# benihime91/pytorch_retinanet

Measured on AMD Instinct MI355X. Metric: images/sec RetinaNet-R50-FPN train step @800x1333, higher is better.
Workload: dtype bf16; 1 GPU; RetinaNet-R50-FPN bf16 train step, per-GPU batch 8 x 3x800x1333 (padded 800x1344), A=201600 anchors, K=90, T=8 GT/img, SGD(momentum, fp32 masters + bf16 conv weights); random-init weights; global_batch=8, parallelism=dp1

## Files before the change

### pytorch_retinanet_amd/csrc/conv.hip

```cpp
#include "rn_common.hpp"
#include <type_traits>
#include <cstdlib>

#ifndef BAND_NARROW_FWD
#define BAND_NARROW_FWD 1
#endif

namespace {

using rn::f32x16;
typedef __attribute__((address_space(3))) void *lds_void_ptr;

constexpr int CONV_BM = 256, CONV_BN = 256, CONV_BK = 64, CONV_THREADS = 512;
constexpr int CONV_LDS_BYTES = 5 * CONV_BM * CONV_BK * 2;
#define SWZ(row) (((row) >> 1) & 7)

constexpr int CONV_MAX_PROBLEMS = 4;

constexpr int CONV_LEVELS = 6;
struct LevelSet {
    const int32_t *map;
    int32_t row_elems, slots, n_images, T;
    int32_t hw[CONV_LEVELS];
    uint16_t *ptr[CONV_LEVELS];
};

__device__ __forceinline__ void sheet_coords(const int m, const int HWp, int &n, int &pos)
{
    n = (int)(((float)m + 0.5f) * (1.0f / (float)HWp));
    pos = m - n * HWp;
}

struct LevelRegs { uint32_t lo[CONV_LEVELS], hi[CONV_LEVELS]; int32_t hw[CONV_LEVELS]; };
__device__ __forceinline__ LevelRegs level_regs(const LevelSet &ls)
{
    LevelRegs r;
#pragma unroll
    for (int l = 0; l < CONV_LEVELS; ++l) {
        const unsigned long long u = (unsigned long long)(uintptr_t)ls.ptr[l];
        r.lo[l] = __builtin_amdgcn_readfirstlane((uint32_t)u);
        r.hi[l] = __builtin_amdgcn_readfirstlane((uint32_t)(u >> 32));
        r.hw[l] = __builtin_amdgcn_readfirstlane(ls.hw[l]);
    }
    return r;
}

__device__ __forceinline__ uint16_t *level_row(const LevelSet &ls, const LevelRegs &lr, const int n, const int32_t e)
{
    if (e < 0) return nullptr;
    const int t = (e >> 24) & 15, img = n * ls.slots + ((e >> 28) & 7), local = e & 0xffffff;
    uint32_t lo = lr.lo[0], hi = lr.hi[0];
    int hw = lr.hw[0];
#pragma unroll
    for (int l = 1; l < CONV_LEVELS; ++l) {
        lo = t == l ? lr.lo[l] : lo;
        hi = t == l ? lr.hi[l] : hi;
        hw = t == l ? lr.hw[l] : hw;
    }
    if (t >= ls.T || img >= ls.n_images || local >= hw) return nullptr;
    uint16_t *base = (uint16_t *)(uintptr_t)(((unsigned long long)hi << 32) | lo);
    return base + ((int64_t)img * hw + local) * ls.row_elems;
}

__device__ __forceinline__ void map_fetch(int32_t &dst, const int32_t *p) { asm volatile("global_load_dword %0, %1, off" : "=v"(dst) : "v"(p) : "memory"); }
__device__ __forceinline__ void map_landed(int32_t &dst) { asm volatile("" : "+v"(dst) :: "memory"); }

__device__ __forceinline__ const uint16_t *bperm_ptr(const uint16_t *p, const int src_lane)
{
    const unsigned long long u = (unsigned long long)(uintptr_t)p;
    unsigned lo, hi;
    const unsigned sel = (unsigned)src_lane << 2;
    asm volatile("ds_bpermute_b32 %0, %2, %3\n\tds_bpermute_b32 %1, %2, %4\n\ts_waitcnt lgkmcnt(0)"
                 : "=&v"(lo), "=&v"(hi) : "v"(sel), "v"((unsigned)u), "v"((unsigned)(u >> 32)) : "memory");
    return (const uint16_t *)(uintptr_t)(((unsigned long long)hi << 32) | lo);
}
template <int LANE_A, int LANE_B>
__device__ __forceinline__ const uint16_t *pair_ptr(const uint16_t *p, const bool second)
{
    const unsigned long long u = (unsigned long long)(uintptr_t)p;
    const unsigned lo_a = __builtin_amdgcn_readlane((unsigned)u, LANE_A), hi_a = __builtin_amdgcn_readlane((unsigned)(u >> 32), LANE_A);
    const unsigned lo_b = __builtin_amdgcn_readlane((unsigned)u, LANE_B), hi_b = __builtin_amdgcn_readlane((unsigned)(u >> 32), LANE_B);
    const unsigned long long a = ((unsigned long long)hi_a << 32) | lo_a, b = ((unsigned long long)hi_b << 32) | lo_b;
    return (const uint16_t *)(uintptr_t)(second ? b : a);
}

enum { MODE_CANVAS = 0, MODE_TO_LEVELS = 1, MODE_FROM_LEVELS = 2, MODE_DENSE = 3 };
struct DenseGeom {
    int64_t M[CONV_MAX_PROBLEMS];
    int32_t h[CONV_MAX_PROBLEMS], w[CONV_MAX_PROBLEMS];
    int32_t tile_beg[CONV_MAX_PROBLEMS + 1];
};

struct ConvArgs {
    const uint16_t *Xs[CONV_MAX_PROBLEMS];
    const uint16_t *Ws[CONV_MAX_PROBLEMS];
    const float *biases[CONV_MAX_PROBLEMS];
    uint16_t *Ys[CONV_MAX_PROBLEMS];
    const uint8_t *mask;
    const uint16_t *zeros;
    const uint8_t *relu_masks[CONV_MAX_PROBLEMS];
    float *colsums[CONV_MAX_PROBLEMS];
    uint8_t *relu_mask_outs[CONV_MAX_PROBLEMS];
    int64_t M, HWp;
    int Cin, Cout, Wp, relu;
    int n_base;
    int f16;
    LevelSet lv;
    DenseGeom dn;
    int ksplit;
    float *kpartial;
    int xcd_ny, xcd_q, xcd_r;
    const uint16_t *X2s[CONV_MAX_PROBLEMS];
    int x_split, x_ld;
};
struct ConvProblem { const uint16_t *X, *W; const float *bias; uint16_t *Y; };

struct Walk { int tap, chunk; };

template <int DT, int MODE, bool NARROW = false>
__global__ __launch_bounds__(CONV_THREADS) void conv3x3_canvas_kernel(const ConvArgs args)
{
    constexpr int MI = NARROW ? 1 : 4;
    int prob = blockIdx.z, bx = blockIdx.x, by = blockIdx.y;
    if (args.xcd_ny > 0) {
        const int xcd = bx & 7, w = bx >> 3, mt = w / args.xcd_ny;
        by = w - mt * args.xcd_ny;
        if (mt >= args.xcd_q + (xcd < args.xcd_r)) return;
        bx = xcd * args.xcd_q + (xcd < args.xcd_r ? xcd : args.xcd_r) + mt;
    }
    int64_t m0 = (int64_t)bx * CONV_BM, M = args.M, HWp = args.HWp;
    int Wp = args.Wp, dense_h = 0;
    if (MODE == MODE_DENSE) {
        prob = 0;
#pragma unroll
        for (int p = 1; p < CONV_MAX_PROBLEMS; ++p) prob = bx >= args.dn.tile_beg[p] ? p : prob;
        m0 = (int64_t)(bx - args.dn.tile_beg[prob]) * CONV_BM;
        M = args.dn.M[prob]; Wp = args.dn.w[prob]; dense_h = args.dn.h[prob]; HWp = (int64_t)Wp * dense_h;
    }
    ConvProblem a;
    a.X = args.Xs[prob]; a.W = args.Ws[prob]; a.bias = args.biases[prob]; a.Y = args.Ys[prob];
    extern __shared__ __attribute__((aligned(16))) unsigned char lds[];
    const int tid = threadIdx.x, lane = tid & 63;
    const int wave = __builtin_amdgcn_readfirstlane(tid >> 6);
    const int wm = NARROW ? wave : wave >> 2, wn = NARROW ? 0 : wave & 3;
    const int grp = wave >> 2;
    const int n0 = by * CONV_BN + args.n_base;
    const int cpt = args.Cin / CONV_BK, KT_ALL = 9 * cpt;
    int kt0 = 0, KT = KT_ALL;
    if (MODE == MODE_DENSE && args.ksplit > 1) {
        const int z = blockIdx.z;
        kt0 = z * KT_ALL / args.ksplit;
        KT = (z + 1) * KT_ALL / args.ksplit - kt0;
    }
    constexpr int TILE = CONV_BM * CONV_BK * 2;
    unsigned char *const Abase = lds, *const Bbase = lds + 3 * TILE;
    auto advance = [&](Walk &w) {
        if (MODE == MODE_FROM_LEVELS) { if (++w.chunk == cpt) { w.chunk = 0; ++w.tap; } }
        else { if (++w.tap == 9) { w.tap = 0; ++w.chunk; } }
    };

    constexpr int MT = 2 * MI, NT = 4;
    rn::f32x4 acc[MT][NT];
#pragma unroll
    for (int i = 0; i < MT; ++i)
#pragma unroll
        for (int j = 0; j < NT; ++j)
#pragma unroll
            for (int r = 0; r < 4; ++r) acc[i][j][r] = 0.0f;

    uint32_t a_off[2], b_off[2];
#pragma unroll
    for (int ks = 0; ks < 2; ++ks) {
        const int chunk = ks * 4 + (lane >> 4);
        { const int row = wm * (32 * MI) + (lane & 15); a_off[ks] = row * 128 + ((chunk ^ SWZ(row)) << 4); }
        { const int row = wn * 64 + (lane & 15); b_off[ks] = row * 128 + ((chunk ^ SWZ(row)) << 4); }
    }
    const uint32_t lds_base = (uint32_t)(uintptr_t)lds;

    const uint16_t *grow[4] = {nullptr, nullptr, nullptr, nullptr};
    LevelRegs lregs = {};
    if (MODE == MODE_TO_LEVELS || MODE == MODE_FROM_LEVELS) lregs = level_regs(args.lv);
    int g_n = 0, g_pos = 0;
    int32_t g_entry = -1;
    bool g_valid = false;
    auto tap_pos = [&](const int t) { return g_pos + (t / 3 - 1) * Wp + (t % 3 - 1); };
    if (MODE == MODE_FROM_LEVELS) {
        const int j = lane & 31;
        int64_t m = m0 + (j >> 3) * 64 + wave * 8 + (j & 7);
        m = m < M ? m : M - 1;
        sheet_coords((int)m, (int)HWp, g_n, g_pos);
        const int p0 = tap_pos(0);
        g_valid = p0 >= 0 && p0 < (int)HWp;
        g_entry = args.lv.map[g_valid ? p0 : 0];
    }
    auto gather_tap = [&](const int t) {
        const uint16_t *mine = level_row(args.lv, lregs, g_n, g_valid ? g_entry : -1);
        const int pn = tap_pos(t + 1 < 9 ? t + 1 : t);
        g_valid = pn >= 0 && pn < (int)HWp;
        map_fetch(g_entry, args.lv.map + (g_valid ? pn : 0));
#pragma unroll
        for (int i = 0; i < 4; ++i) grow[i] = bperm_ptr(mine, i * 8 + (lane >> 3));
    };
    uint32_t voff_a[4], voff_b[4];
#pragma unroll
    for (int i = 0; i < 4; ++i) {
        const int q = i * CONV_THREADS + tid, row = q >> 3, cp = q & 7;
        voff_a[i] = (uint32_t)(row * (MODE == MODE_CANVAS && args.x_split > 0 ? args.x_ld : args.Cin) + ((cp ^ SWZ(row)) << 3)) * 2u;
        voff_b[i] = (uint32_t)(row * 9 * args.Cin + ((cp ^ SWZ(row)) << 3)) * 2u;
    }
    const bool a_edge = m0 - (Wp + 1) < 0 || m0 + CONV_BM + Wp + 1 > M;
    uint32_t tap_ok[4] = {0u, 0u, 0u, 0u};
    if (MODE == MODE_DENSE) {
#pragma unroll
        for (int i = 0; i < 4; ++i) {
            const int64_t m = m0 + ((i * CONV_THREADS + tid) >> 3);
            if (m < M) {
                const int yl = (int)m / Wp, x = (int)m - yl * Wp, y = yl % dense_h;
#pragma unroll
                for (int t = 0; t < 9; ++t)
                    tap_ok[i] |= ((unsigned)(y + t / 3 - 1) < (unsigned)dense_h && (unsigned)(x + t % 3 - 1) < (unsigned)Wp) ? 1u << t : 0u;
            }
        }
    }
    const bool b_ragged = MODE == MODE_TO_LEVELS && n0 + CONV_BN > args.Cout;
    auto lds_piece = [&](unsigned char *stage_base, const int i) {
        return stage_base + i * (CONV_THREADS * 16) + wave * (RN_WAVE * 16);
    };
    auto piece_a = [&](const Walk w, const int stage, const int i) {
        const int c0 = w.chunk * CONV_BK, t = w.tap;
        const int q = i * CONV_THREADS + tid, row = q >> 3, cp = q & 7;
        unsigned char *const sb = Abase + stage * TILE;
        if (MODE == MODE_FROM_LEVELS) {
            const int e = c0 + ((cp ^ SWZ(row)) << 3);
            const int es = e + 8 > args.lv.row_elems ? args.lv.row_elems - 8 : e;
            const uint16_t *g = (grow[i] && e < args.lv.row_elems) ? grow[i] + es : args.zeros + ((cp ^ SWZ(row)) << 3);
            __builtin_amdgcn_global_load_lds((const void *)g, (lds_void_ptr)lds_piece(sb, i), 16, 0, 0);
        } else {
            const int off = (t / 3 - 1) * Wp + (t % 3 - 1);
            if (MODE == MODE_DENSE) {
                const unsigned char *base = (const unsigned char *)a.X + ((m0 + off) * args.Cin + c0) * 2;
                const void *src = (tap_ok[i] >> t) & 1u ? (const void *)(base + voff_a[i]) : (const void *)args.zeros;
                __builtin_amdgcn_global_load_lds(src, (lds_void_ptr)lds_piece(sb, i), 16, 0, 0);
            } else {
                const uint16_t *X = a.X;
                int ld = args.Cin, cs = c0;
                if (MODE == MODE_CANVAS && args.x_split > 0) {
                    ld = args.x_ld;
                    if (w.chunk >= args.x_split) { X = args.X2s[prob]; cs = c0 - args.x_split * CONV_BK; }
                }
                if (!a_edge) {
                    const unsigned char *base = (const unsigned char *)X + ((m0 + off) * ld + cs) * 2;
                    __builtin_amdgcn_global_load_lds((const void *)(base + voff_a[i]), (lds_void_ptr)lds_piece(sb, i), 16, 0, 0);
                } else {
                    int64_t m = m0 + row + off;
                    m = m < 0 ? 0 : (m >= M ? M - 1 : m);
                    const uint16_t *g = X + m * ld + cs + ((cp ^ SWZ(row)) << 3);
                    __builtin_amdgcn_global_load_lds((const void *)g, (lds_void_ptr)lds_piece(sb, i), 16, 0, 0);
                }
            }
        }
    };
    auto piece_b = [&](const Walk w, const int stage, const int i) {
        if (NARROW && i > 0) return;
        const int c0 = w.chunk * CONV_BK, t = w.tap;
        unsigned char *const sb = Bbase + stage * TILE;
        if (!b_ragged) {
            const unsigned char *base = (const unsigned char *)a.W + (((int64_t)n0 * 9 + t) * args.Cin + c0) * 2;
            __builtin_amdgcn_global_load_lds((const void *)(base + voff_b[i]), (lds_void_ptr)lds_piece(sb, i), 16, 0, 0);
        } else {
            const int q = i * CONV_THREADS + tid, row = q >> 3, cp = q & 7;
            const uint16_t *g = a.W + ((int64_t)(n0 + row) * 9 + t) * args.Cin + c0 + ((cp ^ SWZ(row)) << 3);
            if (n0 + row >= args.Cout) g = args.zeros + ((cp ^ SWZ(row)) << 3);
            __builtin_amdgcn_global_load_lds((const void *)g, (lds_void_ptr)lds_piece(sb, i), 16, 0, 0);
        }
    };
    typename rn::mma<DT>::frag fa[MT], fb[NT];
#define RN_DS_READ(dst, addr, OFF) asm volatile("ds_read_b128 %0, %1 offset:" #OFF : "=v"(dst) : "v"(addr))
#define RN_LOAD_FRAGS_AT(AA, KS)                                                   \
    { const uint32_t ba = bbase + b_off[KS], aa = (AA);                            \
      RN_DS_READ(fb[0], ba, 0); RN_DS_READ(fb[1], ba, 2048); RN_DS_READ(fb[2], ba, 4096); RN_DS_READ(fb[3], ba, 6144); \
      RN_DS_READ(fa[0], aa, 0); RN_DS_READ(fa[1], aa, 2048);                        \
      if (MT == 8) { RN_DS_READ(fa[MT - 6], aa, 4096); RN_DS_READ(fa[MT - 5], aa, 6144); RN_DS_READ(fa[MT - 4], aa, 8192);   \
                     RN_DS_READ(fa[MT - 3], aa, 10240); RN_DS_READ(fa[MT - 2], aa, 12288); RN_DS_READ(fa[MT - 1], aa, 14336); } }
#define RN_LOAD_FRAGS(KS) RN_LOAD_FRAGS_AT(abase + a_off[KS], KS)
#define RN_MFMA_ALL()                                                              \
    _Pragma("unroll") for (int mi = 0; mi < MT; ++mi)                              \
        _Pragma("unroll") for (int ni = 0; ni < NT; ++ni)                          \
            acc[mi][ni] = rn::mma<DT>::m16(fa[mi], fb[ni], acc[mi][ni]);
#define RN_MFMA_PHASE()                                                            \
    asm volatile("s_waitcnt lgkmcnt(0)" ::: "memory"); __builtin_amdgcn_sched_barrier(0);          \
    __builtin_amdgcn_s_setprio(1);                                                 \
    RN_MFMA_ALL()                                                                  \
    __builtin_amdgcn_s_setprio(0);                                                 \
    __builtin_amdgcn_sched_barrier(0);                                             \
    __builtin_amdgcn_s_barrier();

    Walk wa = {0, 0}, wb = {0, 0};
    if (MODE == MODE_DENSE) { wa.tap = wb.tap = kt0 % 9; wa.chunk = wb.chunk = kt0 / 9; }
    int sa = 0;
    if (MODE == MODE_FROM_LEVELS) gather_tap(0);
#pragma unroll
    for (int i = 0; i < 4; ++i) piece_a(wa, 0, i);
#pragma unroll
    for (int i = 0; i < 4; ++i) piece_b(wb, 0, i);
    advance(wa); advance(wb);
    if (MODE == MODE_FROM_LEVELS && cpt == 1) {
        asm volatile("s_waitcnt vmcnt(8)" ::: "memory");
        map_landed(g_entry);
        gather_tap(1);
    }
#pragma unroll
    for (int i = 0; i < 4; ++i) piece_a(wa, 1, i);
    advance(wa);
    sa = 2;
    asm volatile("s_waitcnt vmcnt(4)" ::: "memory");
    if (MODE == MODE_FROM_LEVELS) map_landed(g_entry);
    __builtin_amdgcn_s_barrier();
    if (grp == 1) __builtin_amdgcn_s_barrier();


    float bias_pre[4] = {0.0f, 0.0f, 0.0f, 0.0f};
    uint32_t keep[16];
#pragma unroll
    for (int i = 0; i < 16; ++i) keep[i] = 1;
    auto epilogue_prefetch = [&]() {
#pragma unroll
        for (int ni = 0; ni < 4; ++ni) {
            const int col = wn * 64 + ni * 16 + (lane & 15);
            bias_pre[ni] = (a.bias && (MODE != MODE_TO_LEVELS || n0 + col < args.Cout)) ? a.bias[n0 + col] : 0.0f;
        }
        if (MODE != MODE_TO_LEVELS && args.mask) {
            const int64_t pos0 = (int64_t)((uint32_t)m0 % (uint32_t)HWp);
            const bool one_wrap = HWp >= CONV_BM;
#pragma unroll
            for (int i = 0; i < 16; ++i) {
                const int row = i * 16 + (tid >> 5);
                int64_t pos = pos0 + row;
                if (one_wrap) pos = pos >= HWp ? pos - HWp : pos; else pos = (int64_t)((uint32_t)pos % (uint32_t)HWp);
                keep[i] = args.mask[pos];
            }
        }
    };
    int scur = 0;
    for (int kt = 0; kt < KT; ++kt) {
        const uint32_t abase = lds_base + (uint32_t)(scur * TILE), bbase = lds_base + (uint32_t)(3 * TILE + (kt & 1) * TILE);
        scur = scur == 2 ? 0 : scur + 1;
        RN_LOAD_FRAGS(0)
        __builtin_amdgcn_sched_barrier(0);
        if (kt + 1 < KT) {
#pragma unroll
            for (int i = 0; i < 4; ++i) piece_b(wb, (kt + 1) & 1, i);
            advance(wb);
        }
        if (kt == 0) epilogue_prefetch();
        __builtin_amdgcn_sched_barrier(0);
        __builtin_amdgcn_s_barrier();
        RN_MFMA_PHASE()
        RN_LOAD_FRAGS(1)
        __builtin_amdgcn_sched_barrier(0);
        if (kt + 2 < KT) {
            if (MODE == MODE_FROM_LEVELS && wa.chunk == 0) gather_tap(wa.tap);
#pragma unroll
            for (int i = 0; i < 4; ++i) piece_a(wa, sa, i);
            advance(wa);
            sa = sa == 2 ? 0 : sa + 1;
            asm volatile("s_waitcnt vmcnt(4)" ::: "memory");
            if (MODE == MODE_FROM_LEVELS) map_landed(g_entry);
        } else {
            asm volatile("s_waitcnt vmcnt(0)" ::: "memory");
        }
        __builtin_amdgcn_sched_barrier(0);
        __builtin_amdgcn_s_barrier();
        RN_MFMA_PHASE()
    }

#undef RN_DS_READ
#undef RN_LOAD_FRAGS
#undef RN_LOAD_FRAGS_AT
#undef RN_MFMA_ALL
#undef RN_MFMA_PHASE
    if (grp == 0) __builtin_amdgcn_s_barrier();

    if (MODE == MODE_DENSE && args.ksplit > 1) {
        float *__restrict__ out = args.kpartial + ((int64_t)blockIdx.z * M + m0) * args.Cout + n0;
#pragma unroll
        for (int mi = 0; mi < MT; ++mi)
#pragma unroll
            for (int ni = 0; ni < NT; ++ni) {
                const int col = wn * 64 + ni * 16 + (lane & 15);
#pragma unroll
                for (int r = 0; r < 4; ++r) {
                    const int row = wm * (32 * MI) + mi * 16 + 4 * (lane >> 4) + r;
                    if (m0 + row < M) out[(int64_t)row * args.Cout + col] = acc[mi][ni][r];
                }
            }
        return;
    }
    __syncthreads();
    uint16_t *Ys = (uint16_t *)lds;
    uint16_t **Yrow = (uint16_t **)(lds + CONV_BM * CONV_BN * 2);
    float *s_cs = (float *)(lds + CONV_BM * CONV_BN * 2 + 2048);
    uint8_t *s_rmask = lds + CONV_BM * CONV_BN * 2 + 2048 + 16384;
    uint4 *s_lut = (uint4 *)(lds + CONV_BM * CONV_BN * 2 + 2048 + 16384 + 8192);
    static_assert(CONV_BM * CONV_BN * 2 + 2048 + 16384 + 8192 + 4096 <= CONV_LDS_BYTES, "epilogue LDS");
    const uint8_t *relu_mask = MODE == MODE_TO_LEVELS ? nullptr : args.relu_masks[prob];
    uint4 rm_pre = make_uint4(0, 0, 0, 0);
    if (relu_mask) {
        const int row = tid >> 1, half = tid & 1;
        if (m0 + row < M) rm_pre = *(const uint4 *)(relu_mask + (m0 + row) * (args.Cout >> 3) + (n0 >> 3) + half * 16);
    }
    typedef short s16x2 __attribute__((ext_vector_type(2)));
    uint32_t relu_floor = (args.relu & 1) ? 0u : 0x80008000u;
    asm volatile("" : "+v"(relu_floor));
#pragma unroll
    for (int mi = 0; mi < MT; ++mi)
#pragma unroll
        for (int ni = 0; ni < NT; ++ni) {
            const int col = wn * 64 + ni * 16 + (lane & 15);
            const float b = bias_pre[ni];
#pragma unroll
            for (int r = 0; r < 4; r += 2) {
                const int row = wm * (32 * MI) + mi * 16 + 4 * (lane >> 4) + r;
                const float x0 = acc[mi][ni][r] + b, x1 = acc[mi][ni][r + 1] + b;
                uint32_t raw;
                if (DT == RN_BF16) asm("v_cvt_pk_bf16_f32 %0, %1, %2" : "=v"(raw) : "v"(x0), "v"(x1));
                else raw = rn::dt<DT>::pk(x0, x1);
                const uint32_t pk = __builtin_bit_cast(uint32_t, __builtin_elementwise_max(__builtin_bit_cast(s16x2, raw), __builtin_bit_cast(s16x2, relu_floor)));
                Ys[row * CONV_BN + col] = (uint16_t)pk;
                Ys[(row + 1) * CONV_BN + col] = (uint16_t)(pk >> 16);
            }
        }
    if (MODE == MODE_TO_LEVELS && tid < CONV_BM) {
        const int64_t m = m0 + tid;
        uint16_t *dst = nullptr;
        if (m < M) {
            int n, pos;
            sheet_coords((int)m, (int)HWp, n, pos);
            dst = level_row(args.lv, lregs, n, args.lv.map[pos]);
        }
        Yrow[tid] = dst;
    }
    if (relu_mask) {
        *(uint4 *)(s_rmask + tid * 16) = rm_pre;
        if (tid < 256) {
            uint32_t w[4];
#pragma unroll
            for (int j = 0; j < 4; ++j) w[j] = ((tid >> (2 * j)) & 1 ? 0x0000ffffu : 0u) | ((tid >> (2 * j + 1)) & 1 ? 0xffff0000u : 0u);
            s_lut[tid] = make_uint4(w[0], w[1], w[2], w[3]);
        }
    }
    __syncthreads();
    if (MODE == MODE_TO_LEVELS) {
        const int ncols = min(CONV_BN, args.Cout - n0);
#pragma unroll
        for (int i = 0; i < (NARROW ? 4 : 16); ++i) {
            const int q = i * CONV_THREADS + tid, row = NARROW ? q >> 3 : q >> 5, piece = NARROW ? q & 7 : q & 31;
            uint16_t *dst = Yrow[row];
            if (dst && piece * 8 < ncols) {
                const uint16_t *src = Ys + row * CONV_BN + piece * 8;
                dst += n0 + piece * 8;
                if (piece * 8 + 8 <= ncols) {
                    const rn::u32x4 v = *(const rn::u32x4 *)src;
                    asm volatile("global_store_dwordx4 %0, %1, off" :: "v"(dst), "v"(v) : "memory");
                } else {
                    for (int e = 0; e < ncols - piece * 8; e += 2) *(uint32_t *)(dst + e) = *(const uint32_t *)(src + e);
                }
            }
        }
    } else {
        uint8_t *rmask_out = MODE == MODE_TO_LEVELS ? nullptr : args.relu_mask_outs[prob];
        float cs[8] = {0.0f, 0.0f, 0.0f, 0.0f, 0.0f, 0.0f, 0.0f, 0.0f};
#pragma unroll
        for (int i = 0; i < 16; ++i) {
            const int q = i * CONV_THREADS + tid, row = q >> 5, piece = q & 31;
            const int64_t m = m0 + row;
            if (m < M) {
                uint4 v = *(const uint4 *)(Ys + row * CONV_BN + piece * 8);
                if (!keep[i]) v = make_uint4(0, 0, 0, 0);
                if (relu_mask) {
                    const uint4 mk = s_lut[s_rmask[row * 32 + piece]];
                    uint32_t vw[4] = {v.x & mk.x, v.y & mk.y, v.z & mk.z, v.w & mk.w};
#pragma unroll
                    for (int j = 0; j < 4; ++j) {
                        cs[2 * j] += rn::mma<DT>::lo(vw[j]);
                        cs[2 * j + 1] += rn::mma<DT>::hi(vw[j]);
                    }
                    v = make_uint4(vw[0], vw[1], vw[2], vw[3]);
                }
                if (rmask_out) {
                    typedef unsigned short us2 __attribute__((ext_vector_type(2)));
                    const uint32_t vw[4] = {v.x, v.y, v.z, v.w};
                    uint32_t bits = 0;
#pragma unroll
                    for (int j = 0; j < 4; ++j) {
                        const uint32_t nz = __builtin_bit_cast(uint32_t, __builtin_elementwise_min(__builtin_bit_cast(us2, vw[j]), us2{1, 1}));
                        bits |= ((nz | (nz >> 15)) & 3u) << (2 * j);
                    }
                    rmask_out[m * (args.Cout >> 3) + (n0 >> 3) + piece] = (uint8_t)bits;
                }
                *(uint4 *)(a.Y + m * args.Cout + n0 + piece * 8) = v;
            }
        }
        if (relu_mask) {
#pragma unroll
            for (int j = 0; j < 8; ++j) s_cs[(tid >> 5) * CONV_BN + (tid & 31) * 8 + j] = cs[j];
            __syncthreads();
            if (tid < CONV_BN) {
                float t = 0.0f;
#pragma unroll
                for (int r = 0; r < 16; ++r) t += s_cs[r * CONV_BN + tid];
                args.colsums[prob][(int64_t)bx * args.Cout + n0 + tid] = t;
            }
        }
    }
}


constexpr int BAND_BYTES = (CONV_BM + 8) * 128;
constexpr int BANDW_BYTES = 3 * 64 * 128;
constexpr int BAND_LDS = 2 * BAND_BYTES + 2 * BANDW_BYTES;

template <int DT>
__global__ __launch_bounds__(CONV_THREADS) void conv3x3_band_narrow_kernel(const ConvArgs args)
{
    extern __shared__ __attribute__((aligned(16))) unsigned char lds[];
    const int tid = threadIdx.x, lane = tid & 63;
    const int wave = __builtin_amdgcn_readfirstlane(tid >> 6);
    const int64_t m0 = (int64_t)blockIdx.x * CONV_BM, M = args.M;
    const int Wp = args.Wp, cpt = args.Cin / CONV_BK, NB = 3 * cpt;
    const int n0 = args.n_base;
    const uint16_t *__restrict__ X = args.Xs[0], *__restrict__ Wt = args.Ws[0];
    const LevelRegs lregs = level_regs(args.lv);
    const uint32_t lds_base = (uint32_t)(uintptr_t)lds;

    rn::f32x4 acc[2][4];
#pragma unroll
    for (int i = 0; i < 2; ++i)
#pragma unroll
        for (int j = 0; j < 4; ++j)
#pragma unroll
            for (int r = 0; r < 4; ++r) acc[i][j][r] = 0.0f;

    uint32_t a_off[3][2][2], b_off[2];
#pragma unroll
    for (int ks = 0; ks < 2; ++ks) {
        const int chunk = ks * 4 + (lane >> 4);
#pragma unroll
        for (int sft = 0; sft < 3; ++sft)
#pragma unroll
            for (int mi = 0; mi < 2; ++mi) {
                const int row = wave * 32 + mi * 16 + (lane & 15) + sft;
                a_off[sft][mi][ks] = row * 128 + ((chunk ^ SWZ(row)) << 4);
            }
        { const int row = lane & 15; b_off[ks] = row * 128 + ((chunk ^ SWZ(row)) << 4); }
    }

    auto stage = [&](const int b) {
        const int c0 = (b / 3) * CONV_BK, r = b % 3;
        const int64_t p0 = m0 + (int64_t)(r - 1) * Wp - 1;
        unsigned char *const ab = lds + (b & 1) * BAND_BYTES, *const wb = lds + 2 * BAND_BYTES + (b & 1) * BANDW_BYTES;
#pragma unroll
        for (int i = 0; i < 4; ++i) {
            const int q = i * CONV_THREADS + tid, j = q >> 3, cp = q & 7;
            int64_t p = p0 + j;
            p = p < 0 ? 0 : (p >= M ? M - 1 : p);
            const uint16_t *g = X + p * args.Cin + c0 + ((cp ^ SWZ(j)) << 3);
            __builtin_amdgcn_global_load_lds((const void *)g, (lds_void_ptr)(ab + i * (CONV_THREADS * 16) + wave * (RN_WAVE * 16)), 16, 0, 0);
        }
        if (wave == 0) {
            const int j = 256 + (lane >> 3), cp = lane & 7;
            int64_t p = p0 + j;
// ... 878 lines not shown
            rn::dt<DT>::unpack(xv[sr * a.V + j], f0);
#pragma unroll
            for (int e = 0; e < 8; ++e) acc[e] += f0[e];
        }
#pragma unroll
        for (int e = 0; e < 8; ++e) s_acc[(g * a.V + j) * 8 + e] = acc[e];
    }
    __syncthreads();
    const int E = a.V * 8;
    for (int c = t; c < a.C; c += blockDim.x) {
        float tot = 0.0f;
        for (int gg = 0; gg < a.G; ++gg)
            for (int r = 0; r < a.S; ++r) tot += s_acc[gg * E + r * a.C + c];
        if (blockIdx.x == 0)
            for (int64_t row = srows * a.S; row < a.rows[l]; ++row) tot += rn::dt<DT>::ld(x, row * a.C + c);
        a.partial[((int64_t)l * gridDim.x + blockIdx.x) * a.C + c] = tot;
    }
}

__global__ __launch_bounds__(256) void colsum_reduce_kernel(const float *__restrict__ partial, const int tiles, const int C, float *out0,
                                                            float *out1, float *out2, float *out3)
{
    __shared__ double sh[32][8];
    const int p = blockIdx.y, ch = threadIdx.x & 7, ln = threadIdx.x >> 3;
    const int c = blockIdx.x * 8 + ch;
    const float *src = partial + (int64_t)p * tiles * C;
    double s = 0.0;
    if (c < C) {
        int b = ln;
        for (; b + 96 < tiles; b += 128) {
            float v[4];
#pragma unroll
            for (int u = 0; u < 4; ++u) v[u] = src[(int64_t)(b + 32 * u) * C + c];
#pragma unroll
            for (int u = 0; u < 4; ++u) s += (double)v[u];
        }
        for (; b < tiles; b += 32) s += (double)src[(int64_t)b * C + c];
    }
    sh[ln][ch] = s;
    __syncthreads();
    if (ln == 0 && c < C) {
        double t = 0.0;
        for (int l = 0; l < 32; ++l) t += sh[l][ch];
        float *out = p == 0 ? out0 : (p == 1 ? out1 : (p == 2 ? out2 : out3));
        out[c] = (float)t;
    }
}

}

#ifndef CONV_XCD_MAP
#define CONV_XCD_MAP 1
#endif
template <int DT, int MODE, bool NARROW>
static int conv_launch_dt(const ConvArgs &a, const dim3 grid, hipStream_t st)
{
    if (MODE != MODE_DENSE && (a.M >= ((int64_t)1 << 31) || a.HWp >= ((int64_t)1 << 31))) return RN_EUNSUPPORTED;
    static rn::DynLdsOptIn opt_in = {};
    { const int rc = opt_in.ensure((const void *)conv3x3_canvas_kernel<DT, MODE, NARROW>, CONV_LDS_BYTES); if (rc != RN_OK) return rc; }
    if (CONV_XCD_MAP && grid.x >= 16) {
        ConvArgs b = a;
        b.xcd_ny = (int)grid.y; b.xcd_q = (int)(grid.x / 8); b.xcd_r = (int)(grid.x % 8);
        hipLaunchKernelGGL((conv3x3_canvas_kernel<DT, MODE, NARROW>), dim3(8u * (unsigned)(b.xcd_q + (b.xcd_r > 0)) * grid.y, 1, grid.z), dim3(CONV_THREADS),
                           CONV_LDS_BYTES, st, b);
    } else
    hipLaunchKernelGGL((conv3x3_canvas_kernel<DT, MODE, NARROW>), grid, dim3(CONV_THREADS), CONV_LDS_BYTES, st, a);
    RN_LAUNCH_CHECK();
    return RN_OK;
}
template <int MODE, bool NARROW = false>
static int conv_launch_mode(const ConvArgs &a, const dim3 grid, hipStream_t st)
{
    return a.f16 ? conv_launch_dt<RN_F16, MODE, NARROW>(a, grid, st) : conv_launch_dt<RN_BF16, MODE, NARROW>(a, grid, st);
}
static inline bool conv_dtype_ok(const int dtype) { return dtype == RN_BF16 || dtype == RN_F16; }

static int fill_levels(LevelSet &ls, const rn_canvas_layout *lay, int row_elems, void *const *ptrs, int N, int Hp, int Wp)
{
    if (!lay || !lay->map || !ptrs || row_elems <= 0 || (row_elems & 1)) return RN_EINVAL;
    if (lay->T <= 0 || lay->slots <= 0 || lay->n_images <= 0 || (int64_t)N * lay->slots < lay->n_images) return RN_EINVAL;
    if (lay->T > CONV_LEVELS || lay->slots > 8) return RN_EUNSUPPORTED;
    ls.map = lay->map; ls.row_elems = row_elems; ls.slots = lay->slots; ls.n_images = lay->n_images; ls.T = lay->T;
    for (int l = 0; l < CONV_LEVELS; ++l) {
        const int q = l < lay->T ? l : 0;
        if (!ptrs[q] || lay->hw[q] <= 0 || lay->hw[q] >= (1 << 24) || lay->hw[q] > Hp * Wp) return RN_EINVAL;
        if (!rn::aligned(ptrs[q], 16)) return RN_EALIGN;
        if ((int64_t)lay->n_images * lay->hw[q] >= (1ll << 31)) return RN_EUNSUPPORTED;
        ls.hw[l] = lay->hw[q];
        ls.ptr[l] = (uint16_t *)ptrs[q];
    }
    return RN_OK;
}

RN_API int rn_conv3x3_canvas_batched_ex(const void *const *xs, const void *const *ws, const float *const *biases,
                                        const uint8_t *mask, void *const *ys, uint8_t *const *relu_mask_outs, int P, int dtype, int64_t M,
                                        int64_t HWp, int Wp, int Cin, int Cout, int relu, void *stream);

RN_API int rn_conv3x3_canvas_batched(const void *const *xs, const void *const *ws, const float *const *biases,
                                     const uint8_t *mask, void *const *ys, int P, int dtype, int64_t M, int64_t HWp, int Wp,
                                     int Cin, int Cout, int relu, void *stream)
{
    return rn_conv3x3_canvas_batched_ex(xs, ws, biases, mask, ys, nullptr, P, dtype, M, HWp, Wp, Cin, Cout, relu, stream);
}

RN_API int rn_conv3x3_canvas_batched_ex(const void *const *xs, const void *const *ws, const float *const *biases,
                                        const uint8_t *mask, void *const *ys, uint8_t *const *relu_mask_outs, int P, int dtype, int64_t M,
                                        int64_t HWp, int Wp, int Cin, int Cout, int relu, void *stream)
{
    if (relu_mask_outs && !relu) return RN_EINVAL;
    if (!xs || !ws || !ys || P <= 0 || P > CONV_MAX_PROBLEMS || M <= 0 || HWp <= 0 || Wp <= 0 || Cin <= 0 || Cout <= 0) return RN_EINVAL;
    if (!conv_dtype_ok(dtype) || Cin % CONV_BK || Cout % CONV_BN) return RN_EUNSUPPORTED;
    ConvArgs a = {};
    a.f16 = dtype == RN_F16;
    for (int p = 0; p < CONV_MAX_PROBLEMS; ++p) {
        const int q = p < P ? p : 0;
        if (!xs[q] || !ws[q] || !ys[q]) return RN_EINVAL;
        if (!rn::aligned(xs[q], 16) || !rn::aligned(ws[q], 16) || !rn::aligned(ys[q], 16)) return RN_EALIGN;
        a.Xs[p] = (const uint16_t *)xs[q]; a.Ws[p] = (const uint16_t *)ws[q]; a.Ys[p] = (uint16_t *)ys[q];
        a.biases[p] = biases ? biases[q] : nullptr;
        a.relu_mask_outs[p] = relu_mask_outs ? relu_mask_outs[q] : nullptr;
        if (relu_mask_outs && (!relu_mask_outs[q] || !rn::aligned(relu_mask_outs[q], 16))) return relu_mask_outs[q] ? RN_EALIGN : RN_EINVAL;
    }
    a.mask = mask; a.M = M; a.HWp = HWp; a.Cin = Cin; a.Cout = Cout; a.Wp = Wp; a.relu = relu ? 1 : 0; a.zeros = nullptr;
    const dim3 grid((unsigned)((M + CONV_BM - 1) / CONV_BM), (unsigned)(Cout / CONV_BN), (unsigned)P);
    return conv_launch_mode<MODE_CANVAS>(a, grid, (hipStream_t)stream);
}

RN_API int rn_conv3x3_canvas_sum2(const void *x, const void *x2, const void *w, const uint8_t *mask, void *y, int dtype, int64_t M,
                                  int64_t HWp, int Wp, int C, int Cout, void *stream)
{
    if (!x || !x2 || !w || !y || M <= 0 || HWp <= 0 || Wp <= 0 || C <= 0 || Cout <= 0) return RN_EINVAL;
    if (!conv_dtype_ok(dtype) || C % CONV_BK || Cout % CONV_BN) return RN_EUNSUPPORTED;
    if (!rn::aligned(x, 16) || !rn::aligned(x2, 16) || !rn::aligned(w, 16) || !rn::aligned(y, 16)) return RN_EALIGN;
    ConvArgs a = {};
    a.f16 = dtype == RN_F16;
    for (int p = 0; p < CONV_MAX_PROBLEMS; ++p) {
        a.Xs[p] = (const uint16_t *)x; a.X2s[p] = (const uint16_t *)x2; a.Ws[p] = (const uint16_t *)w; a.Ys[p] = (uint16_t *)y;
    }
    a.x_split = C / CONV_BK; a.x_ld = C;
    a.mask = mask; a.M = M; a.HWp = HWp; a.Cin = 2 * C; a.Cout = Cout; a.Wp = Wp; a.relu = 0; a.zeros = nullptr;
    const dim3 grid((unsigned)((M + CONV_BM - 1) / CONV_BM), (unsigned)(Cout / CONV_BN), 1);
    return conv_launch_mode<MODE_CANVAS>(a, grid, (hipStream_t)stream);
}

RN_API int rn_conv3x3_canvas(const void *x, const void *w, const float *bias, const uint8_t *mask, void *y, int dtype,
                             int64_t M, int64_t HWp, int Wp, int Cin, int Cout, int relu, void *stream)
{
    if (!x || !w || !y) return RN_EINVAL;
    const void *xs[1] = {x}, *ws[1] = {w};
    const float *bs[1] = {bias};
    void *ys[1] = {y};
    return rn_conv3x3_canvas_batched(xs, ws, bs, mask, ys, 1, dtype, M, HWp, Wp, Cin, Cout, relu, stream);
}

RN_API int rn_conv3x3_dgrad_weight_batched(const void *const *ws, void *const *outs, int P, int Cout, int Cin, void *stream)
{
    if (!ws || !outs || P <= 0 || P > CONV_MAX_PROBLEMS || Cout <= 0 || Cin <= 0) return RN_EINVAL;
    if (Cout % 32 || Cin % 32) return RN_EUNSUPPORTED;
    WeightPrep a = {};
    for (int p = 0; p < CONV_MAX_PROBLEMS; ++p) {
        const int q = p < P ? p : 0;
        if (!ws[q] || !outs[q] || ws[q] == outs[q]) return RN_EINVAL;
        a.w[p] = (const uint16_t *)ws[q]; a.out[p] = (uint16_t *)outs[q];
    }
    a.Cout = Cout; a.Cin = Cin;
    hipLaunchKernelGGL(dgrad_weight_kernel, dim3((unsigned)(9 * P), (unsigned)(Cout / 32), (unsigned)(Cin / 32)), dim3(256), 0,
                       (hipStream_t)stream, a);
    RN_LAUNCH_CHECK();
    return RN_OK;
}

RN_API int rn_conv3x3_dgrad_weight_many(const void *const *ws, void *const *outs, const int *couts, const int *cins, int n, void *stream)
{
    if (!ws || !outs || !couts || !cins || n <= 0) return RN_EINVAL;
    for (int i0 = 0; i0 < n; i0 += DW_MANY_MAX) {
        WeightPrepMany a = {};
        a.n = n - i0 < DW_MANY_MAX ? n - i0 : DW_MANY_MAX;
        int blocks = 0;
        for (int i = 0; i < a.n; ++i) {
            const int q = i0 + i;
            if (!ws[q] || !outs[q] || ws[q] == outs[q] || couts[q] <= 0 || cins[q] <= 0) return RN_EINVAL;
            if (couts[q] % 32 || cins[q] % 32) return RN_EUNSUPPORTED;
            a.w[i] = (const uint16_t *)ws[q]; a.out[i] = (uint16_t *)outs[q]; a.cout[i] = couts[q]; a.cin[i] = cins[q];
            a.first[i] = blocks;
            blocks += 9 * (couts[q] / 32) * (cins[q] / 32);
        }
        a.first[a.n] = blocks;
        hipLaunchKernelGGL(dgrad_weight_many_kernel, dim3((unsigned)blocks), dim3(256), 0, (hipStream_t)stream, a);
        RN_LAUNCH_CHECK();
    }
    return RN_OK;
}

RN_API int rn_canvas_pack(void *const *levels, const rn_canvas_layout *layout, void *canvas, int dtype, int N, int Hp, int Wp, int C,
                          int to_canvas, void *stream)
// ... 39 lines not shown
    a.G = 1024 / a.V;
    if (a.G > 8) a.G = 8;
    for (int l = 0; l < CONV_LEVELS; ++l) {
        const int q = l < L ? l : 0;
        if (!xs[q] || rows[q] < 0) return RN_EINVAL;
        if (!rn::aligned(xs[q], 16)) return RN_EALIGN;
        a.x[l] = (const uint16_t *)xs[q]; a.rows[l] = rows[q];
    }
    a.partial = (float *)workspace;
    const int threads = ((a.V * a.G + 63) / 64) * 64;
    const size_t lds = (size_t)a.G * a.V * 8 * sizeof(float);
    hipStream_t st = (hipStream_t)stream;
    if (dtype == RN_BF16) hipLaunchKernelGGL((colsum_rows_kernel<RN_BF16>), dim3(CSR_BLOCKS, (unsigned)L), dim3((unsigned)threads), lds, st, a);
    else hipLaunchKernelGGL((colsum_rows_kernel<RN_F16>), dim3(CSR_BLOCKS, (unsigned)L), dim3((unsigned)threads), lds, st, a);
    RN_LAUNCH_CHECK();
    hipLaunchKernelGGL(colsum_reduce_kernel, dim3((unsigned)((C + 7) / 8), 1), dim3(256), 0, st, (const float *)workspace, L * CSR_BLOCKS, C, out,
                       out, out, out);
    RN_LAUNCH_CHECK();
    return RN_OK;
}

RN_API size_t rn_conv3x3_colsum_workspace_bytes(int P, int64_t M, int Cout)
{
    if (P <= 0 || P > CONV_MAX_PROBLEMS || M <= 0 || Cout <= 0) return 0;
    return (size_t)P * (size_t)((M + CONV_BM - 1) / CONV_BM) * (size_t)Cout * sizeof(float);
}

RN_API int rn_conv3x3_canvas_dgrad_relu_batched(const void *const *gs, const void *const *ws, const uint8_t *const *relu_masks,
                                                const uint8_t *mask, void *const *ys, float *const *dbiases, int P, int dtype,
                                                int64_t M, int64_t HWp, int Wp, int Cin, int Cout, void *workspace,
                                                size_t workspace_bytes, void *stream)
{
    if (!gs || !ws || !relu_masks || !ys || !dbiases || !workspace || P <= 0 || P > CONV_MAX_PROBLEMS || M <= 0 || HWp <= 0 || Wp <= 0 ||
        Cin <= 0 || Cout <= 0)
        return RN_EINVAL;
    if (!conv_dtype_ok(dtype) || Cin % CONV_BK || Cout % CONV_BN) return RN_EUNSUPPORTED;
    if (workspace_bytes < rn_conv3x3_colsum_workspace_bytes(P, M, Cout)) return RN_EWORKSPACE;
    ConvArgs a = {};
    a.f16 = dtype == RN_F16;
    const int64_t tiles = (M + CONV_BM - 1) / CONV_BM;
    float *outs[CONV_MAX_PROBLEMS] = {nullptr, nullptr, nullptr, nullptr};
    for (int p = 0; p < CONV_MAX_PROBLEMS; ++p) {
        const int q = p < P ? p : 0;
        if (!gs[q] || !ws[q] || !ys[q] || !relu_masks[q] || !dbiases[q]) return RN_EINVAL;
        if (!rn::aligned(gs[q], 16) || !rn::aligned(ws[q], 16) || !rn::aligned(ys[q], 16) || !rn::aligned(relu_masks[q], 16)) return RN_EALIGN;
        a.Xs[p] = (const uint16_t *)gs[q]; a.Ws[p] = (const uint16_t *)ws[q]; a.Ys[p] = (uint16_t *)ys[q];
        a.biases[p] = nullptr;
        a.relu_masks[p] = relu_masks[q];
        a.colsums[p] = (float *)workspace + (int64_t)q * tiles * Cout;
        outs[p] = dbiases[q];
    }
    a.mask = mask; a.M = M; a.HWp = HWp; a.Cin = Cin; a.Cout = Cout; a.Wp = Wp; a.relu = 0; a.zeros = nullptr;
    const dim3 grid((unsigned)tiles, (unsigned)(Cout / CONV_BN), (unsigned)P);
    const int rc = conv_launch_mode<MODE_CANVAS>(a, grid, (hipStream_t)stream);
    if (rc != RN_OK) return rc;
    hipLaunchKernelGGL(colsum_reduce_kernel, dim3((unsigned)((Cout + 7) / 8), (unsigned)P), dim3(256), 0, (hipStream_t)stream,
                       (const float *)workspace, (int)tiles, Cout, outs[0], outs[1], outs[2], outs[3]);
    RN_LAUNCH_CHECK();
    return RN_OK;
}

RN_API int rn_conv3x3_canvas_to_levels(const void *x, const void *w, const float *bias, const rn_canvas_layout *layout,
                                       void *const *ys, int dtype, int N, int Hp, int Wp, int Cin, int Cout, const void *zeros,
                                       void *stream)
{
    if (!x || !w || !zeros || N <= 0 || Hp <= 2 || Wp <= 2 || Cin <= 0 || Cout <= 0) return RN_EINVAL;
    if (!conv_dtype_ok(dtype) || Cin % CONV_BK || (Cout & 1) || (int64_t)N * Hp * Wp >= (1 << 22)) return RN_EUNSUPPORTED;
    if (!rn::aligned(x, 16) || !rn::aligned(w, 16) || !rn::aligned(zeros, 16)) return RN_EALIGN;
    ConvArgs a = {};
    a.f16 = dtype == RN_F16;
    const int rc = fill_levels(a.lv, layout, Cout, ys, N, Hp, Wp);
    if (rc != RN_OK) return rc;
    for (int p = 0; p < CONV_MAX_PROBLEMS; ++p) { a.Xs[p] = (const uint16_t *)x; a.Ws[p] = (const uint16_t *)w; a.biases[p] = bias; a.Ys[p] = nullptr; }
    a.mask = nullptr; a.M = (int64_t)N * Hp * Wp; a.HWp = (int64_t)Hp * Wp; a.Cin = Cin; a.Cout = Cout; a.Wp = Wp; a.relu = 0;
    a.zeros = (const uint16_t *)zeros;
    const unsigned tiles_m = (unsigned)((a.M + CONV_BM - 1) / CONV_BM);
    const int full = Cout / CONV_BN, rest = Cout % CONV_BN;
    if (rest > 0 && rest <= 64) {
        if (full > 0) {
            const int rc2 = conv_launch_mode<MODE_TO_LEVELS>(a, dim3(tiles_m, (unsigned)full, 1), (hipStream_t)stream);
            if (rc2 != RN_OK) return rc2;
        }
        a.n_base = full * CONV_BN;
        if (BAND_NARROW_FWD) {
            static rn::DynLdsOptIn opt_bf = {}, opt_f = {};
            hipStream_t st = (hipStream_t)stream;
            if (a.f16) {
                const int rc3 = opt_f.ensure((const void *)conv3x3_band_narrow_kernel<RN_F16>, BAND_LDS); if (rc3 != RN_OK) return rc3;
                hipLaunchKernelGGL(conv3x3_band_narrow_kernel<RN_F16>, dim3(tiles_m), dim3(CONV_THREADS), BAND_LDS, st, a);
            } else {
                const int rc3 = opt_bf.ensure((const void *)conv3x3_band_narrow_kernel<RN_BF16>, BAND_LDS); if (rc3 != RN_OK) return rc3;
                hipLaunchKernelGGL(conv3x3_band_narrow_kernel<RN_BF16>, dim3(tiles_m), dim3(CONV_THREADS), BAND_LDS, st, a);
            }
            RN_LAUNCH_CHECK();
            return RN_OK;
        }
        return conv_launch_mode<MODE_TO_LEVELS, true>(a, dim3(tiles_m, 1, 1), (hipStream_t)stream);
    }
    const dim3 grid(tiles_m, (unsigned)((Cout + CONV_BN - 1) / CONV_BN), 1);
    return conv_launch_mode<MODE_TO_LEVELS>(a, grid, (hipStream_t)stream);
}

RN_API int rn_conv3x3_levels_to_canvas(const void *const *gs, const rn_canvas_layout *layout, int row_elems, const void *w,
                                       const uint8_t *mask, void *y, int dtype, int N, int Hp, int Wp, int Kpad, int Cout,
                                       const void *zeros, void *stream)
{
    if (!gs || !w || !y || !zeros || N <= 0 || Hp <= 2 || Wp <= 2 || Kpad <= 0 || Cout <= 0) return RN_EINVAL;
// ... 436 lines not shown
```

Before: 359.3 images/sec.

## Add band-walk A loading to full-width canvas 3x3 conv kernel

Adds a BAND variant of the canvas conv kernel that loads one (BM+8)-row input band per kernel-row and reuses it for the three horizontal taps by shifting the LDS row offset, instead of reloading a separate A tile per tap. This cuts global-to-LDS A traffic roughly threefold for the tower/head convs with Cout=256. The main loop, prefetch schedule and vmcnt waits are restructured, and the keep mask is packed into a bitfield. It is enabled by default via TOWER_BAND for canvas, sum2 and dgrad-colsum launches. It adds complexity in edge clamping and the waitcnt ordering.

```diff
diff --git a/pytorch_retinanet_amd/csrc/conv.hip b/pytorch_retinanet_amd/csrc/conv.hip
--- a/pytorch_retinanet_amd/csrc/conv.hip
+++ b/pytorch_retinanet_amd/csrc/conv.hip
@@ -5,6 +5,9 @@
 #ifndef BAND_NARROW_FWD
 #define BAND_NARROW_FWD 1
 #endif
+#ifndef TOWER_BAND
+#define TOWER_BAND 1
+#endif
 
 namespace {
 
@@ -13,6 +16,7 @@
 
 constexpr int CONV_BM = 256, CONV_BN = 256, CONV_BK = 64, CONV_THREADS = 512;
 constexpr int CONV_LDS_BYTES = 5 * CONV_BM * CONV_BK * 2;
+constexpr int BAND_BYTES = (CONV_BM + 8) * 128;
 #define SWZ(row) (((row) >> 1) & 7)
 
 constexpr int CONV_MAX_PROBLEMS = 4;
@@ -117,9 +121,10 @@
 
 struct Walk { int tap, chunk; };
 
-template <int DT, int MODE, bool NARROW = false>
+template <int DT, int MODE, bool NARROW = false, bool BAND = false>
 __global__ __launch_bounds__(CONV_THREADS) void conv3x3_canvas_kernel(const ConvArgs args)
 {
+    static_assert(!BAND || (MODE == MODE_CANVAS && !NARROW), "the band walk serves the full-width CANVAS mode");
     constexpr int MI = NARROW ? 1 : 4;
     int prob = blockIdx.z, bx = blockIdx.x, by = blockIdx.y;
     if (args.xcd_ny > 0) {
@@ -209,6 +214,17 @@
         voff_b[i] = (uint32_t)(row * 9 * args.Cin + ((cp ^ SWZ(row)) << 3)) * 2u;
     }
     const bool a_edge = m0 - (Wp + 1) < 0 || m0 + CONV_BM + Wp + 1 > M;
+    uint32_t a_off_band[3] = {0u, 0u, 0u}, voff_a4 = 0u, keep_bits = 0xffffu;
+    const bool band_edge = m0 - Wp - 1 < 0 || m0 + Wp - 1 + (CONV_BM + 8) > M;
+    if (BAND) {
+#pragma unroll
+        for (int sft = 0; sft < 3; ++sft) {
+            const int chunk = lane >> 4, row = wm * 128 + (lane & 15) + sft;
+            a_off_band[sft] = row * 128 + ((chunk ^ SWZ(row)) << 4);
+        }
+        const int row = CONV_BM + wave, cp = lane & 7;
+        voff_a4 = (uint32_t)(row * (args.x_split > 0 ? args.x_ld : args.Cin) + ((cp ^ SWZ(row)) << 3)) * 2u;
+    }
     uint32_t tap_ok[4] = {0u, 0u, 0u, 0u};
     if (MODE == MODE_DENSE) {
 #pragma unroll
@@ -266,6 +282,9 @@
         unsigned char *const sb = Bbase + stage * TILE;
         if (!b_ragged) {
             const unsigned char *base = (const unsigned char *)a.W + (((int64_t)n0 * 9 + t) * args.Cin + c0) * 2;
+            if (BAND)
+                __builtin_amdgcn_global_load_lds((const void *)(base + (int64_t)i * (64 * 9 * 2) * args.Cin + voff_b[0]), (lds_void_ptr)lds_piece(sb, i), 16, 0, 0);
+            else
             __builtin_amdgcn_global_load_lds((const void *)(base + voff_b[i]), (lds_void_ptr)lds_piece(sb, i), 16, 0, 0);
         } else {
             const int q = i * CONV_THREADS + tid, row = q >> 3, cp = q & 7;
@@ -274,9 +293,32 @@
             __builtin_amdgcn_global_load_lds((const void *)g, (lds_void_ptr)lds_piece(sb, i), 16, 0, 0);
         }
     };
+    auto piece_band = [&](const Walk w, const int buf, const int i) {
+        if (i == 4 && lane >= 8) return;
+        const uint16_t *X = a.X;
+        int ld = args.Cin, cs = w.chunk * CONV_BK;
+        if (args.x_split > 0) {
+            ld = args.x_ld;
+            if (w.chunk >= args.x_split) { X = args.X2s[prob]; cs -= args.x_split * CONV_BK; }
+        }
+        const int p0 = (int)m0 + (w.tap / 3 - 1) * Wp - 1;
+        unsigned char *const sb = lds + buf * BAND_BYTES;
+        unsigned char *const dst = i < 4 ? lds_piece(sb, i) : sb + (CONV_BM + wave) * 128;
+        const int row0 = i < 4 ? tid >> 3 : CONV_BM + wave;
+        const uint32_t vo = i < 4 ? voff_a[0] : voff_a4;
+        if (!band_edge) {
+            const unsigned char *base = (const unsigned char *)X + (((int64_t)p0 + (i < 4 ? i * 64 : 0)) * ld + cs) * 2;
+            __builtin_amdgcn_global_load_lds((const void *)(base + vo), (lds_void_ptr)dst, 16, 0, 0);
+        } else {
+            int m = p0 + row0 + (i < 4 ? i * 64 : 0);
+            m = m < 0 ? 0 : (m >= (int)M ? (int)M - 1 : m);
+            const uint32_t o = (uint32_t)m * (uint32_t)(ld * 2) + (vo - (uint32_t)row0 * (uint32_t)(ld * 2));
+            __builtin_amdgcn_global_load_lds((const void *)((const unsigned char *)X + cs * 2 + o), (lds_void_ptr)dst, 16, 0, 0);
+        }
+    };
     typename rn::mma<DT>::frag fa[MT], fb[NT];
 #define RN_DS_READ(dst, addr, OFF) asm volatile("ds_read_b128 %0, %1 offset:" #OFF : "=v"(dst) : "v"(addr))
-#define RN_LOAD_FRAGS_AT(AA, KS)                                                   \
+#define RN_LOAD_FRAGS_AT(AA, KS)                                                \
     { const uint32_t ba = bbase + b_off[KS], aa = (AA);                            \
       RN_DS_READ(fb[0], ba, 0); RN_DS_READ(fb[1], ba, 2048); RN_DS_READ(fb[2], ba, 4096); RN_DS_READ(fb[3], ba, 6144); \
       RN_DS_READ(fa[0], aa, 0); RN_DS_READ(fa[1], aa, 2048);                        \
@@ -298,6 +340,14 @@
     Walk wa = {0, 0}, wb = {0, 0};
     if (MODE == MODE_DENSE) { wa.tap = wb.tap = kt0 % 9; wa.chunk = wb.chunk = kt0 / 9; }
     int sa = 0;
+    if (BAND) {
+#pragma unroll
+        for (int i = 0; i < 5; ++i) piece_band(wa, 0, i);
+#pragma unroll
+        for (int i = 0; i < 4; ++i) piece_b(wb, 0, i);
+        wa.tap = 3; advance(wb);
+        asm volatile("s_waitcnt vmcnt(0)" ::: "memory");
+    } else {
     if (MODE == MODE_FROM_LEVELS) gather_tap(0);
 #pragma unroll
     for (int i = 0; i < 4; ++i) piece_a(wa, 0, i);
@@ -315,6 +365,7 @@
     sa = 2;
     asm volatile("s_waitcnt vmcnt(4)" ::: "memory");
     if (MODE == MODE_FROM_LEVELS) map_landed(g_entry);
+    }
     __builtin_amdgcn_s_barrier();
     if (grp == 1) __builtin_amdgcn_s_barrier();
 
@@ -323,7 +374,7 @@
     uint32_t keep[16];
 #pragma unroll
     for (int i = 0; i < 16; ++i) keep[i] = 1;
-    auto epilogue_prefetch = [&]() {
+    auto epilogue_prefetch = [&](uint32_t (&kp)[16]) {
 #pragma unroll
         for (int ni = 0; ni < 4; ++ni) {
             const int col = wn * 64 + ni * 16 + (lane & 15);
@@ -337,10 +388,57 @@
                 const int row = i * 16 + (tid >> 5);
                 int64_t pos = pos0 + row;
                 if (one_wrap) pos = pos >= HWp ? pos - HWp : pos; else pos = (int64_t)((uint32_t)pos % (uint32_t)HWp);
-                keep[i] = args.mask[pos];
+                kp[i] = args.mask[pos];
             }
         }
     };
+    if (BAND) {
+        const int NB = 3 * cpt;
+        for (int b = 0; b < NB; ++b) {
+            const uint32_t aband = lds_base + (uint32_t)((b & 1) * BAND_BYTES);
+            const bool more = b + 1 < NB;
+            uint32_t kp[16];
+#pragma unroll
+            for (int i = 0; i < 16; ++i) kp[i] = 1;
+#pragma unroll
+            for (int sft = 0; sft < 3; ++sft) {
+                const int kt = 3 * b + sft;
+                const uint32_t bbase = lds_base + (uint32_t)(3 * TILE + (kt & 1) * TILE);
+                RN_LOAD_FRAGS_AT(aband + a_off_band[sft], 0)
+                __builtin_amdgcn_sched_barrier(0);
+                if (more || sft < 2) {
+#pragma unroll
+                    for (int i = 0; i < 4; ++i) piece_b(wb, (kt + 1) & 1, i);
+                    advance(wb);
+                }
+                if (sft == 0 && b == 0) epilogue_prefetch(kp);
+                __builtin_amdgcn_sched_barrier(0);
+                __builtin_amdgcn_s_barrier();
+                RN_MFMA_PHASE()
+                RN_LOAD_FRAGS_AT(aband + (a_off_band[sft] ^ 64u), 1)
+                __builtin_amdgcn_sched_barrier(0);
+                if (more && sft == 0) {
+                    piece_band(wa, (b + 1) & 1, 0); piece_band(wa, (b + 1) & 1, 1); piece_band(wa, (b + 1) & 1, 2);
+                    asm volatile("s_waitcnt vmcnt(3)" ::: "memory");
+                    if (b == 0) {
+                        keep_bits = 0u;
+#pragma unroll
+                        for (int i = 0; i < 16; ++i) keep_bits |= kp[i] ? 1u << i : 0u;
+                    }
+                } else if (more && sft == 1) {
+                    piece_band(wa, (b + 1) & 1, 3); piece_band(wa, (b + 1) & 1, 4);
+                    wa.tap += 3;
+                    if (wa.tap == 9) { wa.tap = 0; ++wa.chunk; }
+                    asm volatile("s_waitcnt vmcnt(2)" ::: "memory");
+                } else {
+                    asm volatile("s_waitcnt vmcnt(0)" ::: "memory");
+                }
+                __builtin_amdgcn_sched_barrier(0);
+                __builtin_amdgcn_s_barrier();
+                RN_MFMA_PHASE()
+            }
+        }
+    } else {
     int scur = 0;
     for (int kt = 0; kt < KT; ++kt) {
         const uint32_t abase = lds_base + (uint32_t)(scur * TILE), bbase = lds_base + (uint32_t)(3 * TILE + (kt & 1) * TILE);
@@ -352,7 +450,7 @@
             for (int i = 0; i < 4; ++i) piece_b(wb, (kt + 1) & 1, i);
             advance(wb);
         }
-        if (kt == 0) epilogue_prefetch();
+        if (kt == 0) epilogue_prefetch(keep);
         __builtin_amdgcn_sched_barrier(0);
         __builtin_amdgcn_s_barrier();
         RN_MFMA_PHASE()
@@ -372,6 +470,7 @@
         __builtin_amdgcn_sched_barrier(0);
         __builtin_amdgcn_s_barrier();
         RN_MFMA_PHASE()
+    }
     }
 
 #undef RN_DS_READ
@@ -476,7 +575,7 @@
             const int64_t m = m0 + row;
             if (m < M) {
                 uint4 v = *(const uint4 *)(Ys + row * CONV_BN + piece * 8);
-                if (!keep[i]) v = make_uint4(0, 0, 0, 0);
+                if (BAND ? !((keep_bits >> i) & 1u) : !keep[i]) v = make_uint4(0, 0, 0, 0);
                 if (relu_mask) {
                     const uint4 mk = s_lut[s_rmask[row * 32 + piece]];
                     uint32_t vw[4] = {v.x & mk.x, v.y & mk.y, v.z & mk.z, v.w & mk.w};
@@ -516,7 +615,6 @@
 }
 
 
-constexpr int BAND_BYTES = (CONV_BM + 8) * 128;
 constexpr int BANDW_BYTES = 3 * 64 * 128;
 constexpr int BAND_LDS = 2 * BAND_BYTES + 2 * BANDW_BYTES;
 
@@ -1501,19 +1599,19 @@
 #ifndef CONV_XCD_MAP
 #define CONV_XCD_MAP 1
 #endif
-template <int DT, int MODE, bool NARROW>
+template <int DT, int MODE, bool NARROW, bool BAND = false>
 static int conv_launch_dt(const ConvArgs &a, const dim3 grid, hipStream_t st)
 {
     if (MODE != MODE_DENSE && (a.M >= ((int64_t)1 << 31) || a.HWp >= ((int64_t)1 << 31))) return RN_EUNSUPPORTED;
     static rn::DynLdsOptIn opt_in = {};
-    { const int rc = opt_in.ensure((const void *)conv3x3_canvas_kernel<DT, MODE, NARROW>, CONV_LDS_BYTES); if (rc != RN_OK) return rc; }
+    { const int rc = opt_in.ensure((const void *)conv3x3_canvas_kernel<DT, MODE, NARROW, BAND>, CONV_LDS_BYTES); if (rc != RN_OK) return rc; }
     if (CONV_XCD_MAP && grid.x >= 16) {
         ConvArgs b = a;
         b.xcd_ny = (int)grid.y; b.xcd_q = (int)(grid.x / 8); b.xcd_r = (int)(grid.x % 8);
-        hipLaunchKernelGGL((conv3x3_canvas_kernel<DT, MODE, NARROW>), dim3(8u * (unsigned)(b.xcd_q + (b.xcd_r > 0)) * grid.y, 1, grid.z), dim3(CONV_THREADS),
+        hipLaunchKernelGGL((conv3x3_canvas_kernel<DT, MODE, NARROW, BAND>), dim3(8u * (unsigned)(b.xcd_q + (b.xcd_r > 0)) * grid.y, 1, grid.z), dim3(CONV_THREADS),
                            CONV_LDS_BYTES, st, b);
     } else
-    hipLaunchKernelGGL((conv3x3_canvas_kernel<DT, MODE, NARROW>), grid, dim3(CONV_THREADS), CONV_LDS_BYTES, st, a);
+    hipLaunchKernelGGL((conv3x3_canvas_kernel<DT, MODE, NARROW, BAND>), grid, dim3(CONV_THREADS), CONV_LDS_BYTES, st, a);
     RN_LAUNCH_CHECK();
     return RN_OK;
 }
@@ -1521,6 +1619,13 @@
 static int conv_launch_mode(const ConvArgs &a, const dim3 grid, hipStream_t st)
 {
     return a.f16 ? conv_launch_dt<RN_F16, MODE, NARROW>(a, grid, st) : conv_launch_dt<RN_BF16, MODE, NARROW>(a, grid, st);
+}
+static int conv_launch_canvas(const ConvArgs &a, const dim3 grid, hipStream_t st)
+{
+    const int ld = a.x_split > 0 ? a.x_ld : a.Cin;
+    if (TOWER_BAND && a.Cout == CONV_BN && a.Cin % CONV_BK == 0 && a.M > 0 && (a.M + CONV_BM + 8) * (int64_t)ld * 2 < ((int64_t)1 << 32))
+        return a.f16 ? conv_launch_dt<RN_F16, MODE_CANVAS, false, true>(a, grid, st) : conv_launch_dt<RN_BF16, MODE_CANVAS, false, true>(a, grid, st);
+    return conv_launch_mode<MODE_CANVAS>(a, grid, st);
 }
 static inline bool conv_dtype_ok(const int dtype) { return dtype == RN_BF16 || dtype == RN_F16; }
 
@@ -1572,7 +1677,7 @@
     }
     a.mask = mask; a.M = M; a.HWp = HWp; a.Cin = Cin; a.Cout = Cout; a.Wp = Wp; a.relu = relu ? 1 : 0; a.zeros = nullptr;
     const dim3 grid((unsigned)((M + CONV_BM - 1) / CONV_BM), (unsigned)(Cout / CONV_BN), (unsigned)P);
-    return conv_launch_mode<MODE_CANVAS>(a, grid, (hipStream_t)stream);
+    return conv_launch_canvas(a, grid, (hipStream_t)stream);
 }
 
 RN_API int rn_conv3x3_canvas_sum2(const void *x, const void *x2, const void *w, const uint8_t *mask, void *y, int dtype, int64_t M,
@@ -1589,7 +1694,7 @@
     a.x_split = C / CONV_BK; a.x_ld = C;
     a.mask = mask; a.M = M; a.HWp = HWp; a.Cin = 2 * C; a.Cout = Cout; a.Wp = Wp; a.relu = 0; a.zeros = nullptr;
     const dim3 grid((unsigned)((M + CONV_BM - 1) / CONV_BM), (unsigned)(Cout / CONV_BN), 1);
-    return conv_launch_mode<MODE_CANVAS>(a, grid, (hipStream_t)stream);
+    return conv_launch_canvas(a, grid, (hipStream_t)stream);
 }
 
 RN_API int rn_conv3x3_canvas(const void *x, const void *w, const float *bias, const uint8_t *mask, void *y, int dtype,
@@ -1735,7 +1840,7 @@
     }
     a.mask = mask; a.M = M; a.HWp = HWp; a.Cin = Cin; a.Cout = Cout; a.Wp = Wp; a.relu = 0; a.zeros = nullptr;
     const dim3 grid((unsigned)tiles, (unsigned)(Cout / CONV_BN), (unsigned)P);
-    const int rc = conv_launch_mode<MODE_CANVAS>(a, grid, (hipStream_t)stream);
+    const int rc = conv_launch_canvas(a, grid, (hipStream_t)stream);
     if (rc != RN_OK) return rc;
     hipLaunchKernelGGL(colsum_reduce_kernel, dim3((unsigned)((Cout + 7) / 8), (unsigned)P), dim3(256), 0, (hipStream_t)stream,
                        (const float *)workspace, (int)tiles, Cout, outs[0], outs[1], outs[2], outs[3]);
```

Result: faster. 366.7 images/sec, median of 6 (+2.1%).
